# Justin900429/autonomous_driving_with_diffusion_model

Measured on AMD Instinct MI355X. Metric: denoising-steps/sec, higher is better.
Workload: dtype f32

## Files before the change

### autonomous_driving_with_diffusion_model_amd/_lib.py

```python
from __future__ import annotations

import ctypes as C
import os
from typing import Optional, Sequence

import torch

_HERE = os.path.dirname(os.path.abspath(__file__))
LIB_PATH = os.environ.get("ADX_LIB") or os.path.join(_HERE, "libadx.so")

c_f32p = C.POINTER(C.c_float)
i32, i64, f32, vp = C.c_int32, C.c_int64, C.c_float, C.c_void_p


class TConvDesc(C.Structure):
    _fields_ = [("kind", i32), ("taps", i32), ("stride", i32), ("pad", i32), ("c0", i32), ("c1", i32),
                ("cout", i32), ("lin", i32), ("lout", i32), ("groups", i32), ("eps", f32), ("w_layout", i32),
                ("w_flip", i32), ("exact", i32), ("lin_valid", i32), ("lout_valid", i32)]


class TConvIO(C.Structure):
    _fields_ = [("x0", vp), ("x0_sb", i64), ("x0_sc", i64), ("x0_sl", i64),
                ("x1", vp), ("x1_sb", i64), ("x1_sc", i64), ("x1_sl", i64),
                ("packed_w", vp), ("bias", vp), ("gamma", vp), ("beta", vp),
# ... 151 lines not shown
    "adx_dpm_step": (i32, [C.POINTER(DpmCoef), vp, vp, vp, vp, vp, i32, i32, i32, vp]),
    "adx_traj_select": (i32, [C.POINTER(SelectCfg), vp, vp, vp, vp, vp, vp]),
    "adx_control_state_bytes": (C.c_size_t, [i32, i32, i32]),
    "adx_control_step": (i32, [C.POINTER(ControlCfg), vp, vp, vp, vp, vp, vp]),
    "adx_control_reset": (i32, [vp, i32, i32, i32, vp, vp]),
    "adx_noise_normal": (i32, [vp, i32, i64, vp, i64, vp]),
    "adx_noise_words": (i32, [vp, i32, i64, vp, i64, vp]),
    "adx_noise_advance": (i32, [vp, vp]),
    "adx_warm_init": (i32, [vp, i32, vp, vp, i32, i32, i32, i32, f32, f32, vp, i64, i32, vp]),
    "adx_add_noise": (i32, [vp, vp, vp, vp, vp, i32, vp, i32, i32, i32, i32, vp]),
}

_LAZY_SIGS = {
    "adx_conv2d_pack_ds": (i32, [i32, i32, vp, vp, vp]),
    "adx_conv2d_block_s2_cells": (i32, [i32, i32, vp, vp, vp, vp, vp, vp, vp, vp, vp, i32, i32, i32, i32, vp]),
}

EXPORTED_SYMBOLS = tuple(_SIGS) + tuple(_LAZY_SIGS)

_lib: Optional[C.CDLL] = None


class AdxError(RuntimeError):
    pass


class AdxRangeError(AdxError):

    def __init__(self, groups):
        self.groups = list(groups)
# ... 92 lines not shown
```

### autonomous_driving_with_diffusion_model_amd/csrc/adx_common.h

```cpp
#pragma once
#include <atomic>
#include <mutex>
#include <hip/hip_runtime.h>
#include <stdint.h>
#include <stdio.h>
#include <string.h>

#include "../../include/adx.h"
#include "plan.h"

namespace adx {

void set_error(const char* fmt, ...);

#define ADX_CHECK_HIP(expr)                                                              \
  do {                                                                                   \
    hipError_t _e = (expr);                                                              \
    if (_e != hipSuccess) {                                                              \
      adx::set_error("%s failed: %s (%s:%d)", #expr, hipGetErrorString(_e), __FILE__, __LINE__); \
      return ADX_ERR_HIP;                                                                \
    }                                                                                    \
  } while (0)

#define ADX_REQUIRE(cond, ...)                                                           \
// ... 16 lines not shown
struct DebugSwitches {
  bool conv_exact = false;
  bool wgrad_exact = false;
  bool tconv_exact = false;
  bool unet_chain = true;
  unsigned chain_mask = ~0u;
  bool unet_pipe = true;
  bool conv_vrow = true;
  bool conv_cells = true;
  int train_cells = 5;
  int hs_mode = -1;
  bool wgrad_deterministic = false;
  bool hs_dma = true;
  bool hs_s2q = true;
  bool hs_persist = true;
  int resnet_streams = 2;
  int resnet_split_from = -1;
  bool check_range = false;
};
const DebugSwitches& debug_switches();

struct DeviceOnce {
  std::atomic<uint64_t>& done;
  uint64_t bit = 0;
  bool owner = false;
  static std::mutex& mu() { static std::mutex m; return m; }
  explicit DeviceOnce(std::atomic<uint64_t>& d) : done(d) {
    int dev = 0;
    (void)hipGetDevice(&dev);
    bit = 1ull << (dev & 63);
// ... 46 lines not shown
```

### autonomous_driving_with_diffusion_model_amd/csrc/api.cpp

```cpp
#include <stdarg.h>
#include <stdlib.h>

#include "tconv.h"

namespace adx {

static thread_local char g_err[512] = "";

void set_error(const char* fmt, ...) {
  va_list ap;
  va_start(ap, fmt);
  vsnprintf(g_err, sizeof(g_err), fmt, ap);
  va_end(ap);
}

static thread_local PlanSink* t_plan_sink = nullptr;
PlanSink* plan_sink() { return t_plan_sink; }
void plan_set_sink(PlanSink* s) { t_plan_sink = s; }

int plan_emit(PlanSink* s, const PlanLaunch& l) {
  ADX_REQUIRE(s->n < s->cap, "plan export: more than %d launches", s->cap);
  s->rec[s->n++] = l;
  return ADX_OK;
}
// ... 11 lines not shown
  static const DebugSwitches sw = [] {
    DebugSwitches d;
    auto is = [](const char* name, char v) { const char* e = getenv(name); return e != nullptr && e[0] == v && e[1] == '\0'; };
    d.conv_exact = is("ADX_CONV_EXACT", '1');
    d.wgrad_exact = is("ADX_WGRAD_EXACT", '1');
    d.tconv_exact = is("ADX_TCONV_EXACT", '1');
    d.unet_chain = !is("ADX_UNET_CHAIN", '0');
    d.unet_pipe = !is("ADX_UNET_PIPE", '0');
    d.conv_cells = !is("ADX_CONV_CELLS", '0');
    d.conv_vrow = !is("ADX_CONV_VROW", '0');
    d.train_cells = is("ADX_TRAIN_CELLS", '0') ? 0 : (is("ADX_TRAIN_CELLS", '1') ? 1 : (is("ADX_TRAIN_CELLS", '2') ? 2 : (is("ADX_TRAIN_CELLS", '3') ? 3 : (is("ADX_TRAIN_CELLS", '4') ? 4 : 5))));
    d.check_range = is("ADX_CHECK_RANGE", '1');
    d.hs_dma = !is("ADX_HS_DMA", '0');
    d.hs_persist = !is("ADX_HS_PERSIST", '0');
    d.hs_s2q = !is("ADX_HS_S2Q", '0');
    d.wgrad_deterministic = is("ADX_WGRAD_DETERMINISTIC", '1');
    if (const char* e = getenv("ADX_CHAIN_MASK")) d.chain_mask = (unsigned)strtoul(e, nullptr, 0);
    if (const char* e = getenv("ADX_HS_MODE")) d.hs_mode = atoi(e);
    if (const char* e = getenv("ADX_RESNET_SPLIT_FROM")) d.resnet_split_from = atoi(e) < 0 ? -1 : atoi(e);
    if (const char* e = getenv("ADX_RESNET_STREAMS")) d.resnet_streams = atoi(e) < 1 ? 1 : (atoi(e) > 4 ? 4 : atoi(e));
    return d;
  }();
  return sw;
}

int embed_forward(const adx_embed_weights* w, int dim, const int64_t* t, int t_rows, const float* cond,
                  const float* feat, int feat_rows, int rows, float* time_embed, float* mish_cond, hipStream_t s);
int ddim_step(const adx_step_coef* c, const float* mo, const float* x, const float* z, const float* tgt,
              const float* mask, float* prev, float* x0, int b, int h, int d, hipStream_t s);
int ddpm_step(const adx_step_coef* c, const float* mo, const float* x, const float* z, const float* tgt,
// ... 151 lines not shown
```

### autonomous_driving_with_diffusion_model_amd/csrc/conv2d.hip

```cpp
#include <stdlib.h>

#include <vector>

#include "adx_common.h"
#include "conv2d_internal.h"

namespace adx {

constexpr int kCoutT = 64;
constexpr size_t kMaxLds = 96 * 1024;

template <int STRIDE, int K, int ROWS, int CCH = 16>
__global__ void __launch_bounds__(256) conv2d_kernel(const Conv2dArgs a) {
  constexpr int TH = 4 * ROWS;
  constexpr int CC = (K == 7) ? 4 : CCH;
  constexpr int PH = (TH - 1) * STRIDE + K;
  constexpr int PW = (kTileW - 1) * STRIDE + K;
  constexpr int PLANE = PH * PW;
  constexpr int NP = CC * PLANE;
  constexpr int PITEMS = (NP + 255) / 256;
  constexpr int NTAPS = K * K;
  constexpr int NW4 = NTAPS * CC * (kCoutT / 4);
  constexpr int WITEMS = (NW4 + 255) / 256;
  extern __shared__ __attribute__((aligned(16))) float smem[];
// ... 375 lines not shown
    ADX_REQUIRE(scale == nullptr && relu == 0, "conv2d: BatchNorm-backward statistics belong to data-gradient launches");
    a.bs_raw = bst->raw; a.bs_out = bst->out; a.bs_mean = bst->mean; a.bs_rstd = bst->rstd; a.bs_gamma = bst->gamma;
    a.bs_beta = bst->beta; a.bs_mask = bst->mask; a.bs_bits = bst->mask == 1 ? bst->bits : nullptr;
    a.res_bits = bst->res_bits;
  }
  a.x_cells = (fmt & kFmtXCells) != 0; a.y_cells = (fmt & kFmtYCells) != 0; a.res_cells = (fmt & kFmtResCells) != 0 && res != nullptr;
  Hs3x3Query q;
  q.N = N; q.H = H; q.W = W; q.fmt = fmt;
  q.stats_floats = stats_part != nullptr && stats_p != nullptr ? stats_floats : 0;
  q.bst_mask = a.bs_mask; q.bst_bits = a.bs_bits != nullptr;
  q.x_scale = x_amax == nullptr ? kXScaleNone : (x_amax_n < 0 ? kXScalePre : kXScaleDynamic);
  q.affine = scale != nullptr; q.relu = relu != 0; q.has_res = res != nullptr;
  q.y_aligned = (reinterpret_cast<uintptr_t>(y) & 15) == 0; q.res_aligned = (reinterpret_cast<uintptr_t>(res) & 15) == 0;
  q.split_floats = t_split_floats;
  if (L.k == 3 && L.stride == 1) {
    const int rc = device_cus(&q.cus);
    if (rc != ADX_OK) return rc;
  }
  const Hs3x3Plan plan = conv2d_hs3x3_plan(L, q);
  ADX_REQUIRE(a.res_bits == nullptr || (res != nullptr && L.dgrad && plan.stats == 2),
              "conv2d: a masked residual belongs to a data-gradient launch with the statistics epilogue");
  ADX_REQUIRE(plan.admitted, "conv2d: the cell layout belongs to plain launches of the pipelined 3x3 kernel (%d -> %d, k%d s%d)", L.cin, L.cout,
              L.k, L.stride);
  if (conv2d_hs_eligible(L)) {
    if (plan.stats != 0) {
      a.stats_part = stats_part;
      a.stats_p = plan.stats_tiles;
      *stats_p = plan.stats_tiles;
    }
    return conv2d_hs_launch(L, a, s, &plan);
  }
// ... 83 lines not shown
}

int adx_conv2d_forward_cells(const adx_conv2d_desc* d, const void* x, const float* packed_w, const float* scale,
                             const float* shift, const void* res, void* y, int32_t n, int32_t h, int32_t w, int32_t relu,
                             int32_t fmt, adx_stream stream) {
  ConvSpec L;
  int rc = spec_from_desc(d, &L);
  if (rc != ADX_OK) return rc;
  ADX_REQUIRE(x && packed_w && y, "adx_conv2d_forward_cells: null tensor");
  ADX_REQUIRE((scale == nullptr) == (shift == nullptr), "adx_conv2d_forward_cells: scale and shift go together");
  ADX_REQUIRE(fmt >= 0 && fmt <= 7 && (fmt & kFmtYCells), "adx_conv2d_forward_cells: fmt %d (the output is a cell tensor)", fmt);
  ADX_REQUIRE(conv2d_hs3x3_plain(L, n, h, w), "adx_conv2d_forward_cells: not a plain launch of the pipelined 3x3 kernel "
              "(adx_conv2d_cells_supported)");
  return conv2d_launch_raw(L, (const float*)x, packed_w, scale, shift, (const float*)res, (float*)y, n, h, w, relu,
                           (hipStream_t)stream, nullptr, 0, nullptr, 0, nullptr, fmt);
}

static int block_s2_specs(int32_t cin, int32_t cout, ConvSpec* c1, ConvSpec* ds, const char* who) {
  const adx_conv2d_desc d1{cin, cout, 3, 2, 1}, dd{cin, cout, 1, 2, 0};
  int rc = spec_from_desc(&d1, c1);
  if (rc == ADX_OK) rc = spec_from_desc(&dd, ds);
  if (rc != ADX_OK) return rc;
  ADX_REQUIRE(resnet_fuses_ds(*c1, *ds), "%s: %d -> %d is no block entry the split-fp16 kernels fuse (cin %% 16, cout %% 64, not ADX_CONV_EXACT=1)",
              who, cin, cout);
  return ADX_OK;
}

int adx_conv2d_pack_ds(int32_t cin, int32_t cout, const float* w, float* packed, adx_stream stream) {
  ConvSpec c1, ds;
  const int rc = block_s2_specs(cin, cout, &c1, &ds, "adx_conv2d_pack_ds");
// ... 472 lines not shown
```

### autonomous_driving_with_diffusion_model_amd/csrc/conv2d_hs.hip

```cpp
#include <type_traits>
#include <stdlib.h>

#include "adx_common.h"
#include "conv2d_internal.h"
#include "conv2d_hs_common.h"

namespace adx {

template <bool AFFINE = true>
__device__ __forceinline__ void cells_store32(float (&v)[16], const float* sc, const float* sh, int cl0, const float (*res8)[8],
                                              bool relu, __amdgpu_buffer_rsrc_t yrsrc, uint32_t vcell, uint32_t so, uint32_t cplane,
                                              float& amax) {
  float lm = 0.f;
#pragma unroll
  for (int i = 0; i < 2; ++i)
#pragma unroll
    for (int j = 0; j < 4; ++j) {
      const auto sw = __builtin_amdgcn_permlane32_swap(f2u(v[8 * i + j]), f2u(v[8 * i + 4 + j]), false, false);
      v[8 * i + j] = u2f(sw[0]);
      v[8 * i + 4 + j] = u2f(sw[1]);
    }
#pragma unroll
  for (int i = 0; i < 2; ++i) {
    float o[8];
// ... 1539 lines not shown
  const bool in_ok = (size_t)N * L.cin * q.H * q.W * sizeof(float) < 0xC0000000u;
  const bool bytes_ok = in_ok && (size_t)N * L.cout * OH * OW * sizeof(float) < 0xC0000000u;
  const bool vfits = (long)N * (OW + 1) < (1L << 21);
  const int vw = N > 1 ? OW + 1 : OW;
  const int vtiles_x = (int)(((long)N * vw - (N > 1 ? 1 : 0) + kTileW - 1) / kTileW);
  const bool vrow_ok = sw.conv_vrow && N > 1 && vfits && bytes_ok;
  const bool q_shape = sw.hs_mode < 0 && L.cout % 128 == 0 && L.cin_pad % 64 == 0;
  const bool q_fp32out = q_shape && xc && !yc && !rc && !q.affine && vfits && bytes_ok;
  const bool q_train = q_fp32out && sw.train_cells >= 3 && !q.has_res && q.x_scale == kXScaleNone && q.bst_mask == 0;
  const bool q_dgrad = q_fp32out && sw.train_cells >= 5 && xscaled && !q.relu && (q.bst_mask == 2 || (q.bst_mask == 1 && q.bst_bits));
  const bool q_plain = q_shape && xc && yc && (!q.has_res || rc) && q.x_scale == kXScaleNone;
  const int stats_tiles = q_train || q_dgrad ? ceil_div(OH, kQTH) * vtiles_x
                                             : ceil_div(OH, th) * (!yc && !rc && vrow_ok ? vtiles_x : N * ceil_div(OW, kTileW));
  p.stats_need = (size_t)stats_tiles * (L.cout * 2 + L.cout / 64);
  const bool stats = q.stats_floats > 0 && p.stats_need <= q.stats_floats;
  const bool split_shape = mode == 0 && grid0 <= 64 && nchunks >= 8;
  if (q.fmt == kFmtXCells && q.stats_floats > 0 && q.bst_mask == 0 && q.x_scale == kXScaleNone && sw.train_cells != 0 && !L.dgrad)
    p.admitted = in_ok && stats;
  else if (q.fmt == (kFmtXCells | kFmtXScaled) && L.dgrad && xscaled && sw.train_cells >= 4)
    p.admitted = in_ok;
  else if (q.fmt != 0)
    p.admitted = q.stats_floats == 0 && sw.conv_cells && !L.dgrad && bytes_ok && !split_shape;

  p.family = kHs3x3; p.mode = mode; p.threads = mode == 0 ? 256 : 512;
  p.tiles_x = ceil_div(OW, kTileW); p.tiles_y = ceil_div(OH, th); p.cout_tiles = L.cout / (kHsCout * ct);
  p.vw = OW; p.cper = nchunks;
  p.grid = (size_t)p.cout_tiles * p.tiles_x * p.tiles_y * N;
  if (stats) { p.stats = q.bst_mask != 0 ? 2 : 1; p.stats_tiles = stats_tiles; }
  if (!stats && split_shape && q.split_floats > 0 && q.x_scale == kXScaleNone && (OH * OW) % 4 == 0 && q.y_aligned && (!q.has_res || q.res_aligned)) {
    const size_t out_floats = (size_t)N * L.cout * OH * OW;
    int S = 16;
    while (S > 1 && (nchunks % S != 0 || (nchunks / S) % 2 != 0 || p.grid * S > 256 || out_floats * S > q.split_floats)) S >>= 1;
    if (S > 1) { p.ksplit = S; p.cper = nchunks / S; p.grid *= S; }
  }
  const bool cells_out = !stats && p.ksplit == 1 && (xc || yc || rc) && !(xc && xscaled && !yc && !rc);
  if (stats ? q_train || q_dgrad : cells_out && q_plain) {
    p.family = kHs3x3q; p.dma = sw.hs_dma; p.threads = kQNT;
    p.lds = p.dma ? kQLdsD : kQLds;
    p.vw = vw; p.tiles_x = vtiles_x; p.tiles_y = ceil_div(OH, kQTH); p.cout_tiles = L.cout / 128;
    p.q_slots = ceil_div(p.tiles_x * p.tiles_y, 8);
    if (sw.hs_dma && sw.hs_persist) p.q_slots = std::min(p.q_slots, std::max(1, q.cus / (8 * p.cout_tiles)));
    p.grid = (size_t)8 * p.cout_tiles * p.q_slots;
    return p;
  }
  p.lds = hs3x3_lds(mode, p.stats);
  if (p.ksplit > 1) return p;
  p.xcells = xc; p.ycells = cells_out;
  p.vr = !cells_out && (!(xc || yc || rc) || ((stats || xscaled) && !yc && !rc)) && vrow_ok;
  if (p.ycells || p.vr) {
    p.vw = vw; p.tiles_x = vtiles_x;
// ... 101 lines not shown
  a.KH = 2; a.KW = 2; a.stride = 1; a.pad = 0; a.relu = 0;
  a.cin_pad = cout; a.cc = kHsCC;
  a.d2s_cin = cin; a.d2s_h = H; a.d2s_w = W;
  ADX_REQUIRE((size_t)cin * H * W * sizeof(float) < 0x7FFFFFFFu, "conv2d_hs_dgrad_s2: one image of dx exceeds the 32-bit byte offsets");
  return hs_launch_t<1, 2, 2, 2, false>(a, s);
}

int conv2d_hs_launch(const ConvSpec& L, Conv2dArgs a, hipStream_t s, const Hs3x3Plan* plan) {
  ADX_REQUIRE((size_t)L.cin * a.H * a.W * sizeof(float) < 0xC0000000u, "conv2d_hs: one image of the input exceeds the 32-bit byte offsets");
  const bool ds = a.w_ds != nullptr;
  if (hs_is_stem(L) && !ds) {
    ADX_REQUIRE(a.x_amax == nullptr && a.res == nullptr, "conv2d_hs stem: no residual / dynamic range");
    return hs_stem_launch(a, s);
  }
  if (L.k == 3 && L.stride == 1 && !ds) {
    if (plan != nullptr && plan->family != kHsNone) return plan->family == kHs3x3q ? conv2d_hs3x3q_launch(*plan, a, s) : hs3x3_launch(*plan, a, s);
    ADX_REQUIRE(a.stats_part == nullptr, "conv2d_hs: statistics requested from a launch the pipelined kernel does not serve");
    return hs_launch_t<1, 3, 2, 2, false>(a, s);
  }
  if (L.k == 3 && L.stride == 2 && L.pad == 1) {
    if (a.x_cells || a.y_cells) {
      ADX_REQUIRE(ds && a.x_amax == nullptr && a.res == nullptr && a.d2s_cin == 0,
                  "conv2d_hs: cell-layout operands of the stride-2 conv need the fused downsample launch (no residual, no dynamic range)");
      if (a.x_cells && a.y_cells) return hs_launch_t<2, 3, 1, 1, true, true, true>(a, s);
      return a.x_cells ? hs_launch_t<2, 3, 1, 1, true, true, false>(a, s) : hs_launch_t<2, 3, 1, 1, true, false, true>(a, s);
    }
    return ds ? hs_launch_t<2, 3, 1, 1, true>(a, s) : hs_launch_t<2, 3, 1, 1, false>(a, s);
  }
  set_error("conv2d_hs: no kernel for k=%d stride=%d pad=%d%s", L.k, L.stride, L.pad, ds ? " with a fused downsample" : "");
  return ADX_ERR_INVALID;
// ... 10 lines not shown
```

### autonomous_driving_with_diffusion_model_amd/csrc/conv2d_hs16.hip

```cpp
#include "adx_common.h"
#include "conv2d_internal.h"
#include "conv2d_hs_common.h"

namespace adx {

namespace {

typedef __attribute__((address_space(3))) void lds_void;

__device__ __forceinline__ f32x4 mfma16(f16x8 a, f16x8 b, f32x4 c) { return __builtin_amdgcn_mfma_f32_16x16x32_f16(a, b, c, 0, 0, 0); }

__device__ __forceinline__ void half4(uint32_t h0, uint32_t h1, uint32_t l0, uint32_t l1, float* out) {
  const float inv = 1.f / kLoScale;
  asm("v_fma_mix_f32 %0, %1, %2, %3 op_sel:[0,0,0] op_sel_hi:[1,0,1]" : "=v"(out[0]) : "v"(l0), "s"(inv), "v"(h0));
  asm("v_fma_mix_f32 %0, %1, %2, %3 op_sel:[1,0,1] op_sel_hi:[1,0,1]" : "=v"(out[1]) : "v"(l0), "s"(inv), "v"(h0));
  asm("v_fma_mix_f32 %0, %1, %2, %3 op_sel:[0,0,0] op_sel_hi:[1,0,1]" : "=v"(out[2]) : "v"(l1), "s"(inv), "v"(h1));
  asm("v_fma_mix_f32 %0, %1, %2, %3 op_sel:[1,0,1] op_sel_hi:[1,0,1]" : "=v"(out[3]) : "v"(l1), "s"(inv), "v"(h1));
}

}

template <bool DMA, int TRAIN = 0>
__global__ void __launch_bounds__(kQNT, 2) conv2d_hs3x3q_kernel(const Conv2dArgs a) {
  constexpr bool S2 = TRAIN == 3;
// ... 565 lines not shown
      const uint32_t so = cell0 + (uint32_t)(2 * cb) * 2u * cplane;
      __builtin_amdgcn_raw_buffer_store_b128(hi, yrsrc, vcell[rr], so, 0);
      __builtin_amdgcn_raw_buffer_store_b128(lo, yrsrc, vcell[rr], so + cplane, 0);
      asm volatile("s_nop 0" ::"v"(hi), "v"(lo));
    }
  bad |= ((vcell[0] != kOutside) & out_of_fp16(am[0])) | ((vcell[1] != kOutside) & out_of_fp16(am[1]));
  } while (S2 && ++pass < 2);
  }
  if (!has_next) break;
  if constexpr (TRAIN == 1 || TRAIN == 2) __syncthreads();
  sp = sp_next; tx = ntx; ty = nty; oy0 = n_oy0; vx0 = n_vx0;
  }
  range_flag(a.status, bad);
}

int conv2d_hs3x3q_launch(const Hs3x3Plan& p, Conv2dArgs a, hipStream_t s) {
  typedef void (*QKernel)(const Conv2dArgs);
  static const QKernel table[2][3] = {
      {&conv2d_hs3x3q_kernel<false, 0>, &conv2d_hs3x3q_kernel<false, 1>, &conv2d_hs3x3q_kernel<false, 2>},
      {&conv2d_hs3x3q_kernel<true, 0>, &conv2d_hs3x3q_kernel<true, 1>, &conv2d_hs3x3q_kernel<true, 2>}};
  static std::atomic<uint64_t> attr{0};
  if (DeviceOnce once{attr}; once) {
    for (int dma = 0; dma < 2; ++dma)
      for (const QKernel k : table[dma])
        ADX_CHECK_HIP(hipFuncSetAttribute(reinterpret_cast<const void*>(k), hipFuncAttributeMaxDynamicSharedMemorySize, (int)(dma ? kQLdsD : kQLds)));
    once.commit();
  }
  ADX_REQUIRE((long)a.N * p.vw < (1L << 21), "conv2d_hs: batch x width exceeds the virtual-row arithmetic");
  const size_t tiles = (size_t)p.cout_tiles * p.tiles_x * p.tiles_y;
  ADX_REQUIRE(tiles < (1u << 31), "conv2d_hs: grid too large");
// ... 13 lines not shown
  if (DeviceOnce once{attr}; once) {
    ADX_CHECK_HIP(hipFuncSetAttribute(reinterpret_cast<const void*>(&conv2d_hs3x3q_kernel<true, 3>), hipFuncAttributeMaxDynamicSharedMemorySize, (int)kQLdsS2));
    once.commit();
  }
  ADX_REQUIRE(p.q && a.x_cells && a.y_cells && a.w_ds != nullptr && a.y_ds != nullptr && a.res == nullptr && a.x_amax == nullptr,
              "conv2d_hs: the 16x16x32 block entry takes a cell input, two cell outputs, no residual and no dynamic range");
  a.vw = p.vw; a.inv_vw = 1.f / (float)p.vw;
  a.tiles_x = p.tiles_x; a.tiles_y = p.tiles_y; a.cout_tiles = p.cout_tiles; a.ntiles = p.cout_tiles * p.tiles_x * p.tiles_y;
  a.q_slots = p.q_slots;
  a.ksplit = 1; a.cper = a.cin_pad / kHsCC; a.part = nullptr;
  conv2d_hs3x3q_kernel<true, 3><<<dim3((unsigned)p.grid), dim3(p.threads), p.lds, s>>>(a);
  ADX_LAUNCH_CHECK();
  return ADX_OK;
}

}
```

### autonomous_driving_with_diffusion_model_amd/csrc/conv2d_hs_common.h

```cpp
#pragma once
#include "adx_common.h"

namespace adx {

typedef _Float16 f16x8 __attribute__((ext_vector_type(8)));
typedef uint32_t u32x4 __attribute__((ext_vector_type(4)));
typedef _Float16 f16x2 __attribute__((ext_vector_type(2)));

constexpr int kHsCout = 64;
constexpr int kHsCC = 16;
constexpr float kLoScale = 2048.f;

constexpr int kQNT = 512;
constexpr int kQTH = 8;
constexpr int kQPW = 34;
constexpr int kQPlane = (kQTH + 2) * kQPW;
constexpr int kQPlaneP = 344;
constexpr int kQPairs = 4 * kQPlane;
constexpr int kQPit = (kQPairs + kQNT - 1) / kQNT;
constexpr int kQWst = 1024;
constexpr size_t kQLds = (size_t)2 * 8 * kQPlaneP * 16 + (size_t)2 * kQWst * 16 + 256 * sizeof(float) + 2 * 16 + 512 * sizeof(float);
constexpr int kQPlaneD = 352;
constexpr int kQPairsD = 4 * kQPlaneD;
constexpr size_t kQLdsD = (size_t)2 * 8 * kQPlaneD * 16 + (size_t)2 * kQWst * 16 + 256 * sizeof(float) + 2 * 16 + 512 * sizeof(float) +
                          (size_t)kQPit * kQNT * sizeof(uint32_t);
constexpr size_t kQLdsS2 = kQLdsD + (size_t)4 * kQPit * kQNT * sizeof(uint32_t);
static_assert(kQLds <= 160 * 1024 && kQLdsD <= 160 * 1024 && kQLdsS2 <= 160 * 1024, "LDS budget");

#ifdef ADX_HS_M16_TIMING
typedef float f32x4_t __attribute__((ext_vector_type(4)));
__device__ __forceinline__ f32x16 hs_mfma(f16x8 a, f16x8 b, f32x16 c) {
  f32x4_t c0 = __builtin_shufflevector(c, c, 0, 1, 2, 3), c1 = __builtin_shufflevector(c, c, 4, 5, 6, 7);
  c0 = __builtin_amdgcn_mfma_f32_16x16x32_f16(a, b, c0, 0, 0, 0);
  c1 = __builtin_amdgcn_mfma_f32_16x16x32_f16(a, b, c1, 0, 0, 0);
  c[0] = c0[0]; c[1] = c0[1]; c[2] = c0[2]; c[3] = c0[3];
  c[4] = c1[0]; c[5] = c1[1]; c[6] = c1[2]; c[7] = c1[3];
  return c;
}
#else
__device__ __forceinline__ f32x16 hs_mfma(f16x8 a, f16x8 b, f32x16 c) { return __builtin_amdgcn_mfma_f32_32x32x16_f16(a, b, c, 0, 0, 0); }
#endif

// ... 20 lines not shown
```

### autonomous_driving_with_diffusion_model_amd/csrc/conv2d_internal.h

```cpp
#pragma once
#include <vector>

#include "adx_common.h"

namespace adx {

constexpr int kTileH = 4;
constexpr int kTileW = 32;

struct ConvSpec {
  int cin, cout, k, stride, pad;
  int t_w, t_g, t_b, t_m, t_v;
  size_t o_w, o_scale, o_shift;
  int cin_pad, cc;
  int fuse_with;
  int dgrad;
};

struct Conv2dArgs {
  const float* x;
  const float* w;
  const float* scale;
  const float* shift;
  const float* res;
// ... 45 lines not shown
  hipStream_t side[kMaxSub - 1] = {nullptr, nullptr, nullptr};
  hipEvent_t ev_fork = nullptr, ev_join[kMaxSub - 1] = {nullptr, nullptr, nullptr};
  int side_device = -1;
  uint32_t* status = nullptr;
};

namespace adx {

struct BnBwdStats { const float* raw; const float* out; const float* mean; const float* rstd; const float* gamma; const float* beta; int mask;
                    const uint8_t* bits = nullptr; const uint8_t* res_bits = nullptr; };
int conv2d_launch_raw(const ConvSpec& L, const float* x, const float* w, const float* scale, const float* shift,
                      const float* res, float* y, int N, int H, int W, int relu, hipStream_t s,
                      const uint32_t* x_amax = nullptr, int x_amax_n = 0, float* stats_part = nullptr, size_t stats_floats = 0,
                      int* stats_p = nullptr, int fmt = 0, const BnBwdStats* bst = nullptr);

enum { kHsNone = 0, kHs3x3 = 1, kHs3x3q = 2 };
enum { kXScaleNone = 0, kXScaleDynamic = 1, kXScalePre = 2 };
struct Hs3x3Query {
  int N = 0, H = 0, W = 0;
  int fmt = 0;
  size_t stats_floats = 0;
  int bst_mask = 0;
  bool bst_bits = false;
  int x_scale = kXScaleNone;
  bool affine = false, relu = false, has_res = false;
  bool y_aligned = true, res_aligned = true;
  size_t split_floats = 0;
  int cus = 0;
};
struct Hs3x3Plan {
  bool admitted = false;
  int family = kHsNone;
  int mode = 0;
  int stats = 0;
  bool xcells = false, ycells = false, vr = false;
  bool dma = false;
  int ksplit = 1, cper = 0;
  int tiles_x = 0, tiles_y = 0, cout_tiles = 0, vw = 0, q_slots = 0;
  size_t grid = 0;
  int threads = 0;
  size_t lds = 0;
  int stats_tiles = 0;
  size_t stats_need = 0;
// ... 20 lines not shown
  q.fmt = x_cells ? kFmtXCells | kFmtXScaled : 0;
  q.x_scale = x_cells ? kXScalePre : kXScaleDynamic;
  const Hs3x3Plan p = conv2d_hs3x3_plan(L, q);
  return L.dgrad && p.admitted && p.stats == 2;
}
int conv2d_pack_raw(const float* w, float* packed, int cout, int cin, int k, int cin_pad, int dgrad, hipStream_t s);
int conv2d_pack_spec(const ConvSpec& consumer, const float* w, float* packed, int dgrad, hipStream_t s);
bool conv2d_hs_eligible(const ConvSpec& L, const DebugSwitches& sw = debug_switches());
size_t conv2d_packed_floats(const ConvSpec& L);
int conv2d_hs_pack(const ConvSpec& consumer, const float* w, void* packed, int dgrad, hipStream_t s);
struct HsPackJob { const float* w; void* packed; int cout, cin_pad, cin, taps, dgrad; };
bool conv2d_hs_pack_batchable(const ConvSpec& consumer, int dgrad);
int conv2d_hs_pack_many(const HsPackJob* jobs, int n, hipStream_t s);
int conv2d_hs_launch(const ConvSpec& L, Conv2dArgs a, hipStream_t s, const Hs3x3Plan* plan = nullptr);
int conv2d_hs3x3q_launch(const Hs3x3Plan& p, Conv2dArgs a, hipStream_t s);
bool conv2d_hs_dgrad_s2_eligible(int cin, int cout);
int conv2d_hs_dgrad_s2(const float* w, const float* dy, float* dx, int accumulate, int N, int cin, int cout, int H, int W,
                       float* wbuild, float* wimg, const uint32_t* dy_amax, int dy_amax_n, hipStream_t s);
void conv2d_set_split_scratch(float* p, size_t floats);
void conv2d_set_status(uint32_t* word);
uint32_t* conv2d_status();
int conv2d_hs_stem_pool(const ConvSpec& L, const float* x, const float* w, const float* scale, const float* shift,
                        float* pooled, int N, int H, int W, hipStream_t s, const uint8_t* frames_u8 = nullptr,
                        const float* mean = nullptr, const float* stdv = nullptr, int y_cells = 0);
int conv2d_hs_launch_block_s2(const ConvSpec& c1, const ConvSpec& ds, const float* x, const float* w1, const float* scale1,
                              const float* shift1, float* y1, const float* wd, const float* scaled, const float* shiftd,
                              float* yd, int N, int H, int W, hipStream_t s, int x_cells = 0, int y_cells = 0, int relu = 1,
                              bool force_32 = false);
struct HsS2Query {
  int N = 0, H = 0, W = 0;
// ... 74 lines not shown
```

### include/adx.h

```cpp
#ifndef ADX_H
#define ADX_H

#include <stddef.h>
#include <stdint.h>

#ifdef __cplusplus
extern "C" {
#endif

#define ADX_OK 0
#define ADX_ERR_INVALID (-1)
#define ADX_ERR_HIP (-2)
#define ADX_ERR_STATE (-3)
#define ADX_ERR_RANGE (-4)

typedef void* adx_stream;

int adx_version(void);
const char* adx_source_hash(void);
const char* adx_last_error(void);


typedef struct adx_tconv_desc {
  int32_t kind, taps, stride, pad;
// ... 134 lines not shown
                             int32_t max_records);
int32_t adx_resnet_status_words(const adx_resnet* r);
int adx_resnet_set_status(adx_resnet* r, uint32_t* words );
const char* adx_resnet_status_name(const adx_resnet* r, int32_t group);

typedef struct adx_conv2d_desc { int32_t cin, cout, k, stride, pad; } adx_conv2d_desc;
size_t adx_conv2d_packed_bytes(const adx_conv2d_desc* d);
int adx_conv2d_pack(const adx_conv2d_desc* d, const float* w , float* packed, adx_stream s);
int adx_conv2d_forward(const adx_conv2d_desc* d, const float* x, const float* packed_w, const float* scale,
                       const float* shift, const float* res, float* y, int32_t n, int32_t h, int32_t w,
                       int32_t relu, adx_stream s);
int adx_conv2d_cells_supported(const adx_conv2d_desc* d, int32_t n, int32_t h, int32_t w);
int adx_conv2d_forward_cells(const adx_conv2d_desc* d, const void* x, const float* packed_w, const float* scale,
                             const float* shift, const void* res, void* y, int32_t n, int32_t h, int32_t w, int32_t relu,
                             int32_t fmt, adx_stream s);
int adx_conv2d_pack_ds(int32_t cin, int32_t cout, const float* w, float* packed, adx_stream s);
int adx_conv2d_block_s2_cells(int32_t cin, int32_t cout, const void* x, const float* packed_w1, const float* scale1,
                              const float* shift1, void* y1, const float* packed_wd, const float* scaled, const float* shiftd,
                              void* yd, int32_t n, int32_t h, int32_t w, int32_t flags, adx_stream s);
int adx_conv2d_stem_pool(const void* x, int32_t x_u8, const float* packed_w, const float* scale, const float* shift,
                         const float* mean, const float* stdv, void* y, int32_t n, int32_t h, int32_t w, int32_t y_cells,
                         adx_stream s);
size_t adx_conv2d_wgrad_scratch_bytes(void);
int adx_conv2d_wgrad(const adx_conv2d_desc* d, const float* x, const float* dy, float* dw, int32_t n, int32_t h,
                     int32_t w, void* scratch, adx_stream s);
int adx_conv2d_wgrad_ex(const adx_conv2d_desc* d, const float* x, const float* dy, float* dw, int32_t n, int32_t h,
                        int32_t w, void* scratch, int32_t estimate_range, adx_stream s);
int adx_conv2d_wgrad_cells(const adx_conv2d_desc* d, const void* x_cells, const void* dy_cells, const float* dy_scale, float* dw,
                           int32_t n, int32_t h, int32_t w, void* scratch, adx_stream s);

// ... 167 lines not shown
```

Before: 167.2.

## Add 4-wave two-workgroups-per-CU 3x3 cell conv kernel variant

Adds a new 256-thread form of the fp16-split 3x3 stride-1 cell-layout convolution. It uses a smaller LDS footprint so two workgroups fit per CU, and each workgroup computes 64 output channels with a persistent tile loop that prefetches the next tile's patch. The planner picks it for plain all-cell inference launches with enough tiles, based on a queried occupancy. A plan-query API is also exposed. The aim is better latency hiding and CU utilisation on the ResNet perception convs, at the cost of another kernel path with different tiling.

```diff
diff --git a/autonomous_driving_with_diffusion_model_amd/_lib.py b/autonomous_driving_with_diffusion_model_amd/_lib.py
--- a/autonomous_driving_with_diffusion_model_amd/_lib.py
+++ b/autonomous_driving_with_diffusion_model_amd/_lib.py
@@ -189,6 +189,7 @@
 _LAZY_SIGS = {
     "adx_conv2d_pack_ds": (i32, [i32, i32, vp, vp, vp]),
     "adx_conv2d_block_s2_cells": (i32, [i32, i32, vp, vp, vp, vp, vp, vp, vp, vp, vp, i32, i32, i32, i32, vp]),
+    "adx_conv2d_cells_plan": (i32, [i32, i32, i32, i32, i32, i32, i32, i32, C.POINTER(i32)]),
 }
 
 EXPORTED_SYMBOLS = tuple(_SIGS) + tuple(_LAZY_SIGS)
diff --git a/autonomous_driving_with_diffusion_model_amd/csrc/adx_common.h b/autonomous_driving_with_diffusion_model_amd/csrc/adx_common.h
--- a/autonomous_driving_with_diffusion_model_amd/csrc/adx_common.h
+++ b/autonomous_driving_with_diffusion_model_amd/csrc/adx_common.h
@@ -54,6 +54,7 @@
   bool hs_dma = true;
   bool hs_s2q = true;
   bool hs_persist = true;
+  int hs_q64 = 1;
   int resnet_streams = 2;
   int resnet_split_from = -1;
   bool check_range = false;
diff --git a/autonomous_driving_with_diffusion_model_amd/csrc/api.cpp b/autonomous_driving_with_diffusion_model_amd/csrc/api.cpp
--- a/autonomous_driving_with_diffusion_model_amd/csrc/api.cpp
+++ b/autonomous_driving_with_diffusion_model_amd/csrc/api.cpp
@@ -49,6 +49,7 @@
     d.hs_dma = !is("ADX_HS_DMA", '0');
     d.hs_persist = !is("ADX_HS_PERSIST", '0');
     d.hs_s2q = !is("ADX_HS_S2Q", '0');
+    d.hs_q64 = is("ADX_HS_Q64", '0') ? 0 : (is("ADX_HS_Q64", '2') ? 2 : 1);
     d.wgrad_deterministic = is("ADX_WGRAD_DETERMINISTIC", '1');
     if (const char* e = getenv("ADX_CHAIN_MASK")) d.chain_mask = (unsigned)strtoul(e, nullptr, 0);
     if (const char* e = getenv("ADX_HS_MODE")) d.hs_mode = atoi(e);
diff --git a/autonomous_driving_with_diffusion_model_amd/csrc/conv2d.hip b/autonomous_driving_with_diffusion_model_amd/csrc/conv2d.hip
--- a/autonomous_driving_with_diffusion_model_amd/csrc/conv2d.hip
+++ b/autonomous_driving_with_diffusion_model_amd/csrc/conv2d.hip
@@ -413,7 +413,8 @@
   q.y_aligned = (reinterpret_cast<uintptr_t>(y) & 15) == 0; q.res_aligned = (reinterpret_cast<uintptr_t>(res) & 15) == 0;
   q.split_floats = t_split_floats;
   if (L.k == 3 && L.stride == 1) {
-    const int rc = device_cus(&q.cus);
+    int rc = device_cus(&q.cus);
+    if (rc == ADX_OK && debug_switches().hs_q64 != 0) rc = conv2d_hs3x3q64_wgs_per_cu(&q.q64_wgs_per_cu);
     if (rc != ADX_OK) return rc;
   }
   const Hs3x3Plan plan = conv2d_hs3x3_plan(L, q);
@@ -527,6 +528,25 @@
               "(adx_conv2d_cells_supported)");
   return conv2d_launch_raw(L, (const float*)x, packed_w, scale, shift, (const float*)res, (float*)y, n, h, w, relu,
                            (hipStream_t)stream, nullptr, 0, nullptr, 0, nullptr, fmt);
+}
+
+int adx_conv2d_cells_plan(int32_t cin, int32_t cout, int32_t n, int32_t h, int32_t w, int32_t has_res, int32_t cus,
+                          int32_t wgs_per_cu, int32_t* ints) {
+  ADX_REQUIRE(ints != nullptr && n >= 1 && h >= 1 && w >= 1 && cus >= 1 && wgs_per_cu >= 0, "adx_conv2d_cells_plan: bad argument");
+  const adx_conv2d_desc d{cin, cout, 3, 1, 1};
+  ConvSpec L;
+  const int rc = spec_from_desc(&d, &L);
+  if (rc != ADX_OK) return rc;
+  Hs3x3Query q;
+  q.N = n; q.H = h; q.W = w; q.has_res = has_res != 0;
+  q.fmt = kFmtXCells | kFmtYCells | (has_res ? kFmtResCells : 0);
+  q.cus = cus > 8 ? cus : 8; q.q64_wgs_per_cu = wgs_per_cu;
+  const Hs3x3Plan p = conv2d_hs3x3_plan(L, q);
+  const bool cell_launch = p.admitted && p.family != kHsNone;
+  const int32_t v[ADX_CONV3X3_PLAN_INTS] = {cell_launch ? p.family : kHsNone, p.mode, p.threads, (int32_t)p.grid, p.q_slots, (int32_t)p.lds,
+                                            p.tiles_x, p.tiles_y, p.cout_tiles};
+  for (int i = 0; i < ADX_CONV3X3_PLAN_INTS; ++i) ints[i] = cell_launch ? v[i] : 0;
+  return ADX_OK;
 }
 
 static int block_s2_specs(int32_t cin, int32_t cout, ConvSpec* c1, ConvSpec* ds, const char* who) {
diff --git a/autonomous_driving_with_diffusion_model_amd/csrc/conv2d_hs.hip b/autonomous_driving_with_diffusion_model_amd/csrc/conv2d_hs.hip
--- a/autonomous_driving_with_diffusion_model_amd/csrc/conv2d_hs.hip
+++ b/autonomous_driving_with_diffusion_model_amd/csrc/conv2d_hs.hip
@@ -1577,7 +1577,10 @@
                                              : ceil_div(OH, th) * (!yc && !rc && vrow_ok ? vtiles_x : N * ceil_div(OW, kTileW));
   p.stats_need = (size_t)stats_tiles * (L.cout * 2 + L.cout / 64);
   const bool stats = q.stats_floats > 0 && p.stats_need <= q.stats_floats;
-  const bool split_shape = mode == 0 && grid0 <= 64 && nchunks >= 8;
+  const bool q64_scope = sw.hs_q64 != 0 && sw.hs_mode < 0 && sw.hs_dma && sw.conv_cells && L.cout % 64 == 0 && L.cin_pad % 64 == 0 && !L.dgrad &&
+                         q.stats_floats == 0 && xc && yc && (!q.has_res || rc) && q.x_scale == kXScaleNone && bytes_ok && vfits;
+  const bool q64_forced = sw.hs_q64 == 2 && q64_scope;
+  const bool split_shape = mode == 0 && grid0 <= 64 && nchunks >= 8 && !q64_forced;
   if (q.fmt == kFmtXCells && q.stats_floats > 0 && q.bst_mask == 0 && q.x_scale == kXScaleNone && sw.train_cells != 0 && !L.dgrad)
     p.admitted = in_ok && stats;
   else if (q.fmt == (kFmtXCells | kFmtXScaled) && L.dgrad && xscaled && sw.train_cells >= 4)
@@ -1597,6 +1600,16 @@
     if (S > 1) { p.ksplit = S; p.cper = nchunks / S; p.grid *= S; }
   }
   const bool cells_out = !stats && p.ksplit == 1 && (xc || yc || rc) && !(xc && xscaled && !yc && !rc);
+  const long q64_tiles = (long)vtiles_x * ceil_div(OH, kQTH) * (L.cout / 64);
+  if (q64_scope && p.ksplit == 1 && q.q64_wgs_per_cu >= 2 && (q64_forced || (!q_plain && q64_tiles >= 2L * q.cus))) {
+    p.family = kHs3x3q64; p.dma = true; p.threads = kQ64NT;
+    p.lds = kQ64Lds;
+    p.vw = vw; p.tiles_x = vtiles_x; p.tiles_y = ceil_div(OH, kQTH); p.cout_tiles = L.cout / 64;
+    p.q_slots = ceil_div(p.tiles_x * p.tiles_y, 8);
+    if (sw.hs_persist) p.q_slots = std::min(p.q_slots, std::max(1, q.q64_wgs_per_cu * q.cus / (8 * p.cout_tiles)));
+    p.grid = (size_t)8 * p.cout_tiles * p.q_slots;
+    return p;
+  }
   if (stats ? q_train || q_dgrad : cells_out && q_plain) {
     p.family = kHs3x3q; p.dma = sw.hs_dma; p.threads = kQNT;
     p.lds = p.dma ? kQLdsD : kQLds;
@@ -1728,6 +1741,7 @@
     return hs_stem_launch(a, s);
   }
   if (L.k == 3 && L.stride == 1 && !ds) {
+    if (plan != nullptr && plan->family == kHs3x3q64) return conv2d_hs3x3q64_launch(*plan, a, s);
     if (plan != nullptr && plan->family != kHsNone) return plan->family == kHs3x3q ? conv2d_hs3x3q_launch(*plan, a, s) : hs3x3_launch(*plan, a, s);
     ADX_REQUIRE(a.stats_part == nullptr, "conv2d_hs: statistics requested from a launch the pipelined kernel does not serve");
     return hs_launch_t<1, 3, 2, 2, false>(a, s);
diff --git a/autonomous_driving_with_diffusion_model_amd/csrc/conv2d_hs16.hip b/autonomous_driving_with_diffusion_model_amd/csrc/conv2d_hs16.hip
--- a/autonomous_driving_with_diffusion_model_amd/csrc/conv2d_hs16.hip
+++ b/autonomous_driving_with_diffusion_model_amd/csrc/conv2d_hs16.hip
@@ -603,6 +603,236 @@
   range_flag(a.status, bad);
 }
 
+namespace q64 {
+
+template <bool DMA, int TRAIN = 0>
+__global__ void __launch_bounds__(kQ64NT, 2) conv2d_hs3x3q_kernel(const Conv2dArgs a) {
+  static_assert(DMA && TRAIN == 0, "the 4-wave form serves the LDS-DMA inference launch only");
+  constexpr int NT = kQ64NT, PW = kQPW, PLANE = kQPlaneD, PP = kQPlaneD, PIT = kQ64Pit, WST = kQ64Wst, NPAIRS = kQPairsD;
+  constexpr int GST = PP, PLST = 4 * PP;
+  extern __shared__ __attribute__((aligned(16))) unsigned char smem_raw[];
+  u32x4* patch = reinterpret_cast<u32x4*>(smem_raw);
+  u32x4* wl = patch + 8 * PP;
+  float* ss = reinterpret_cast<float*>(wl + 2 * WST);
+  u32x4* dummy = reinterpret_cast<u32x4*>(ss + 128);
+  uint32_t* gnext = reinterpret_cast<uint32_t*>(dummy + 2);
+  const int tid = threadIdx.x, lane = tid & 63;
+  const int rowpair = __builtin_amdgcn_readfirstlane(tid >> 6);
+  const int j = lane & 15, kq = lane >> 4;
+  const int Qs = a.q_slots;
+  const int xcd = blockIdx.x & 7, rr_ = blockIdx.x >> 3;
+  const int ct = rr_ % a.cout_tiles, slot = rr_ / a.cout_tiles;
+  const int nsp = a.tiles_x * a.tiles_y;
+  const int sp_end = (int)(((long)(xcd + 1) * nsp) >> 3);
+  int sp = (int)(((long)xcd * nsp) >> 3) + slot;
+  if (sp >= sp_end) return;
+  int ty = sp / a.tiles_x, tx = sp - ty * a.tiles_x;
+  int oy0 = ty * kQTH, vx0 = tx * 32;
+  auto vdiv = [&](int v) { return (int)(((float)v + 0.5f) * a.inv_vw); };
+  const size_t hw = (size_t)a.H * a.W;
+  const int nch16 = a.cin_pad / 16, nch32 = a.cin_pad / 32, nstages = nch32 * 9;
+  constexpr uint32_t kOutside = 0xC0000000u;
+  const __amdgpu_buffer_rsrc_t xrsrc = __builtin_amdgcn_make_buffer_rsrc(
+      const_cast<float*>(a.x), 0, (int)(uint32_t)((size_t)a.N * a.Cin * hw * sizeof(float)), 0x00020000);
+  const uint32_t plane_bytes = (uint32_t)(hw * sizeof(float));
+  auto goff_of = [&](int t_, int k, int oy0_, int vx0_) -> uint32_t {
+    const int e = t_ + NT * k;
+    const int g = e / PLANE, p = e - g * PLANE;
+    const int py = p / PW, px = p - py * PW;
+    const int iy = oy0_ - 1 + py;
+    const int v = vx0_ - 1 + px;
+    const int ni = vdiv(v < 0 ? 0 : v);
+    const int ix = v - ni * a.vw;
+    const bool ok = e < NPAIRS && p < kQPlane && iy >= 0 && iy < a.H && ix >= 0 && ix < a.W && ni < a.N;
+    return !ok ? kOutside : (uint32_t)((size_t)ni * a.Cin * hw * sizeof(float) + (size_t)g * 8 * hw * sizeof(float) + ((size_t)iy * a.W + ix) * 16);
+  };
+  uint32_t goff[PIT];
+#pragma unroll
+  for (int k = 0; k < PIT; ++k) goff[k] = goff_of(tid, k, oy0, vx0);
+  const u32x4* wsrc = reinterpret_cast<const u32x4*>(a.w);
+  int wsrc_off[2];
+#pragma unroll
+  for (int k = 0; k < 2; ++k) wsrc_off[k] = ((ct * nch16 + k) * 9) * 256 + tid;
+  float ssv = 0.f;
+  if (tid < 128) {
+    const int c = ct * 64 + (tid & 63);
+    ssv = a.scale == nullptr ? (tid < 64 ? 1.f : 0.f) : (tid < 64 ? a.scale[c] : a.shift[c]);
+  }
+
+  f32x4 accm[4][4], accl[4][4];
+
+  const int wcell = __builtin_amdgcn_readfirstlane(tid & ~63);
+  auto load_w = [&](int stage, int buf) {
+    const int chunk = stage / 9, tap = stage - chunk * 9;
+    const u32x4* ws = wsrc + (size_t)(chunk * 18 + tap) * 256;
+#pragma unroll
+    for (int k = 0; k < 2; ++k) __builtin_amdgcn_global_load_lds(ws + wsrc_off[k], (lds_void*)(wl + buf * WST + wcell + NT * k), 16, 0, 0);
+  };
+  auto load_p_at = [&](int chunk, int k, uint32_t go) {
+    const uint32_t cbase = (uint32_t)chunk * 32u * plane_bytes;
+    if (k < PIT - 1 || wcell + NT * k < NPAIRS) {
+      u32x4* d = patch + wcell + NT * k;
+      __builtin_amdgcn_raw_ptr_buffer_load_lds(xrsrc, (lds_void*)d, 16, go, cbase, 0, 0);
+      __builtin_amdgcn_raw_ptr_buffer_load_lds(xrsrc, (lds_void*)(d + PLST), 16, go, cbase + 4 * plane_bytes, 0, 0);
+    }
+  };
+
+  load_w(0, 0);
+#pragma unroll
+  for (int k = 0; k < PIT; ++k) load_p_at(0, k, goff[k]);
+  if (tid < 128) ss[tid] = ssv;
+  asm volatile("s_waitcnt vmcnt(0)" ::: "memory");
+  __syncthreads();
+
+  bool bad = false;
+  for (;;) {
+  int zero_ = 0;
+  asm volatile("" : "+s"(zero_));
+  const int tl = tid + zero_;
+#pragma unroll
+  for (int k = 0; k < PIT; ++k) goff[k] = goff_of(tl, k, oy0, vx0);
+#pragma unroll
+  for (int k = 0; k < 2; ++k) wsrc_off[k] = ((ct * nch16 + k) * 9) * 256 + tl;
+  const int j_l = tl & 15, kq_l = (tl & 63) >> 4;
+  const int pb_lane = kq_l * GST + (rowpair * 2) * PW + j_l;
+  const int wa_lane = (kq_l >> 1) * 256 + (kq_l & 1) * 64 + j_l;
+  const int sp_next = sp + Qs;
+  const bool has_next = sp_next < sp_end;
+  const int nty = sp_next / a.tiles_x, ntx = sp_next - nty * a.tiles_x;
+  const int n_oy0 = nty * kQTH, n_vx0 = ntx * 32;
+  if (has_next) {
+#pragma unroll
+    for (int k = 0; k < PIT; ++k) gnext[k * NT + tid] = goff_of(tl, k, n_oy0, n_vx0);
+  }
+#pragma unroll
+  for (int cb = 0; cb < 4; ++cb)
+#pragma unroll
+    for (int pb = 0; pb < 4; ++pb)
+#pragma unroll
+      for (int i = 0; i < 4; ++i) { accm[cb][pb][i] = 0.f; accl[cb][pb][i] = 0.f; }
+
+  for (int cp = 0; cp < nch32; cp += 2) {
+#pragma unroll
+    for (int i = 0; i < 18; ++i) {
+      const int s = 9 * cp + i;
+      const int cpar = i / 9, t = i % 9, kh = t / 3, kw = t % 3;
+      const u32x4* pb0 = patch + pb_lane + kh * PW + kw;
+      const u32x4* wa0 = wl + (i & 1) * WST + wa_lane;
+      load_w(s + 1 < nstages ? s + 1 : (has_next ? 0 : nstages - 1), (i + 1) & 1);
+      __builtin_amdgcn_sched_barrier(0);
+      f16x8 A[2][4], B[2][4];
+#pragma unroll
+      for (int pl = 0; pl < 2; ++pl) {
+#pragma unroll
+        for (int cb = 0; cb < 4; ++cb) A[pl][cb] = __builtin_bit_cast(f16x8, wa0[pl * 128 + cb * 16]);
+#pragma unroll
+        for (int pb = 0; pb < 4; ++pb) B[pl][pb] = __builtin_bit_cast(f16x8, pb0[pl * PLST + (pb >> 1) * PW + (pb & 1) * 16]);
+      }
+#pragma unroll
+      for (int pb = 0; pb < 4; ++pb) {
+#pragma unroll
+        for (int cb = 0; cb < 4; ++cb) {
+          accm[cb][pb] = mfma16(A[0][cb], B[0][pb], accm[cb][pb]);
+          accl[cb][pb] = mfma16(A[0][cb], B[1][pb], accl[cb][pb]);
+        }
+#pragma unroll
+        for (int cb = 0; cb < 4; ++cb) accl[cb][pb] = mfma16(A[1][cb], B[0][pb], accl[cb][pb]);
+      }
+      asm volatile("s_waitcnt vmcnt(0)" ::: "memory");
+      __syncthreads();
+      if (t == 8) {
+        const bool tile_end = cpar == 1 && cp + 2 >= nch32;
+        if (!tile_end) {
+#pragma unroll
+          for (int k = 0; k < PIT; ++k) load_p_at(cp + cpar + 1, k, goff[k]);
+          asm volatile("s_waitcnt vmcnt(0)" ::: "memory");
+          __syncthreads();
+        } else if (has_next) {
+#pragma unroll
+          for (int k = 0; k < PIT; ++k) load_p_at(0, k, gnext[k * NT + tid]);
+        }
+      }
+    }
+  }
+
+  {
+  const int rw = kq;
+  const int vcol = vx0 + 16 * (rw & 1) + j;
+  const int nl = vdiv(vcol), xl = vcol - nl * a.vw;
+  const bool col_valid = nl < a.N && xl < a.W;
+  const uint32_t plane_ob = (uint32_t)(a.OH * a.OW) * (uint32_t)sizeof(float);
+  const uint32_t cplane = (uint32_t)(a.OH * a.OW) * 16u;
+  const uint32_t img_bytes = (uint32_t)a.N * (uint32_t)a.Cout * plane_ob;
+  const uint32_t img_off = (uint32_t)nl * (uint32_t)a.Cout * plane_ob;
+  const __amdgpu_buffer_rsrc_t yrsrc = __builtin_amdgcn_make_buffer_rsrc(a.y, 0, (int)img_bytes, 0x00020000);
+  const __amdgpu_buffer_rsrc_t rrsrc = __builtin_amdgcn_make_buffer_rsrc(
+      const_cast<float*>(a.res != nullptr ? a.res : a.y), 0, a.res != nullptr ? (int)img_bytes : 0, 0x00020000);
+  const int cout0 = ct * 64;
+  const uint32_t cell0 = (uint32_t)(cout0 >> 3) * 2u * cplane;
+  uint32_t vcell[2];
+#pragma unroll
+  for (int rr = 0; rr < 2; ++rr) {
+    const int oy = oy0 + rowpair * 2 + rr;
+    vcell[rr] = (col_valid && oy < a.OH) ? img_off + (uint32_t)(oy * a.OW + xl) * 16u + (uint32_t)(rw >> 1) * 2u * cplane : kOutside;
+  }
+  u32x4 rh[4][2], rl[4][2];
+#pragma unroll
+  for (int cb = 0; cb < 4; ++cb)
+#pragma unroll
+    for (int rr = 0; rr < 2; ++rr) {
+      const uint32_t so = cell0 + (uint32_t)(2 * cb) * 2u * cplane;
+      rh[cb][rr] = __builtin_amdgcn_raw_buffer_load_b128(rrsrc, vcell[rr], so, 0);
+      rl[cb][rr] = __builtin_amdgcn_raw_buffer_load_b128(rrsrc, vcell[rr], so + cplane, 0);
+    }
+  const float* sc = ss;
+  const float* sh = ss + 64;
+  float am[2] = {0.f, 0.f};
+#pragma unroll
+  for (int cb = 0; cb < 4; ++cb)
+#pragma unroll
+    for (int rr = 0; rr < 2; ++rr) {
+      float x[4], y[4];
+#pragma unroll
+      for (int i = 0; i < 4; ++i) {
+        const int cl = cb * 16 + 4 * kq + i;
+        x[i] = (accm[cb][2 * rr][i] + accl[cb][2 * rr][i] * (1.f / kLoScale)) * sc[cl] + sh[cl];
+        y[i] = (accm[cb][2 * rr + 1][i] + accl[cb][2 * rr + 1][i] * (1.f / kLoScale)) * sc[cl] + sh[cl];
+      }
+      float o[8];
+#pragma unroll
+      for (int i = 0; i < 4; ++i) {
+        const auto sw = __builtin_amdgcn_permlane16_swap(f2u(x[i]), f2u(y[i]), false, false);
+        o[i] = u2f(sw[0]);
+        o[4 + i] = u2f(sw[1]);
+      }
+      float r8[8];
+      half4(rh[cb][rr][0], rh[cb][rr][1], rl[cb][rr][0], rl[cb][rr][1], r8);
+      half4(rh[cb][rr][2], rh[cb][rr][3], rl[cb][rr][2], rl[cb][rr][3], r8 + 4);
+#pragma unroll
+      for (int i = 0; i < 8; ++i) {
+        const float tsum = o[i] + r8[i];
+        o[i] = a.relu ? __builtin_fmaxf(tsum, 0.f) : tsum;
+        am[rr] = fp16_amax(am[rr], o[i]);
+      }
+      u32x4 hi, lo;
+      split8(o, 1.f, hi, lo);
+      const uint32_t so = cell0 + (uint32_t)(2 * cb) * 2u * cplane;
+      __builtin_amdgcn_raw_buffer_store_b128(hi, yrsrc, vcell[rr], so, 0);
+      __builtin_amdgcn_raw_buffer_store_b128(lo, yrsrc, vcell[rr], so + cplane, 0);
+      asm volatile("s_nop 0" ::"v"(hi), "v"(lo));
+    }
+  bad |= ((vcell[0] != kOutside) & out_of_fp16(am[0])) | ((vcell[1] != kOutside) & out_of_fp16(am[1]));
+  }
+  if (!has_next) break;
+  asm volatile("s_waitcnt vmcnt(0)" ::: "memory");
+  __syncthreads();
+  sp = sp_next; tx = ntx; ty = nty; oy0 = n_oy0; vx0 = n_vx0;
+  }
+  range_flag(a.status, bad);
+}
+
+}
+
 int conv2d_hs3x3q_launch(const Hs3x3Plan& p, Conv2dArgs a, hipStream_t s) {
   typedef void (*QKernel)(const Conv2dArgs);
   static const QKernel table[2][3] = {
@@ -646,4 +876,43 @@
   return ADX_OK;
 }
 
+static std::atomic<uint64_t> g_q64_once{0};
+static std::atomic<int> g_q64_wgs[64];
+int conv2d_hs3x3q64_wgs_per_cu(int* wgs) {
+  int dev = 0;
+  ADX_CHECK_HIP(hipGetDevice(&dev));
+  if (DeviceOnce once{g_q64_once}; once) {
+    const void* k = reinterpret_cast<const void*>(&q64::conv2d_hs3x3q_kernel<true, 0>);
+    ADX_CHECK_HIP(hipFuncSetAttribute(k, hipFuncAttributeMaxDynamicSharedMemorySize, (int)kQ64Lds));
+    int n = 0;
+    ADX_CHECK_HIP(hipOccupancyMaxActiveBlocksPerMultiprocessor(&n, k, kQ64NT, kQ64Lds));
+    g_q64_wgs[dev & 63].store(n, std::memory_order_relaxed);
+    once.commit();
+  }
+  *wgs = g_q64_wgs[dev & 63].load(std::memory_order_relaxed);
+  return ADX_OK;
 }
+
+int conv2d_hs3x3q64_launch(const Hs3x3Plan& p, Conv2dArgs a, hipStream_t s) {
+  int wgs = 0;
+  const int rc = conv2d_hs3x3q64_wgs_per_cu(&wgs);
+  if (rc != ADX_OK) return rc;
+  ADX_REQUIRE(p.family == kHs3x3q64 && p.dma && p.stats == 0 && a.x_cells && a.y_cells && (a.res == nullptr || a.res_cells) && a.x_amax == nullptr &&
+                  a.Cout % 64 == 0 && a.cin_pad % 64 == 0 && a.Cin == a.cin_pad,
+              "conv2d_hs: the 4-wave 16x16x32 form takes plain all-cell launches with Cout %% 64 == 0 and Cin %% 64 == 0");
+  ADX_REQUIRE((long)a.N * p.vw < (1L << 21), "conv2d_hs: batch x width exceeds the virtual-row arithmetic");
+  const size_t tiles = (size_t)p.cout_tiles * p.tiles_x * p.tiles_y;
+  ADX_REQUIRE(tiles < (1u << 31) && p.cout_tiles == a.Cout / 64 && p.q_slots >= 1 && p.grid == (size_t)8 * p.cout_tiles * p.q_slots,
+              "conv2d_hs: inconsistent plan of the 4-wave 16x16x32 form");
+  ADX_REQUIRE((size_t)a.N * a.Cout * a.OH * a.OW * sizeof(float) < 0xC0000000u && (size_t)a.N * a.Cin * a.H * a.W * sizeof(float) < 0xC0000000u,
+              "conv2d_hs: a cell-layout tensor exceeds the 32-bit byte offsets");
+  a.vw = p.vw; a.inv_vw = 1.f / (float)p.vw;
+  a.tiles_x = p.tiles_x; a.tiles_y = p.tiles_y; a.cout_tiles = p.cout_tiles; a.ntiles = (int)tiles;
+  a.q_slots = p.q_slots;
+  a.ksplit = 1; a.cper = a.cin_pad / kHsCC; a.part = nullptr;
+  q64::conv2d_hs3x3q_kernel<true, 0><<<dim3((unsigned)p.grid), dim3(p.threads), p.lds, s>>>(a);
+  ADX_LAUNCH_CHECK();
+  return ADX_OK;
+}
+
+}
diff --git a/autonomous_driving_with_diffusion_model_amd/csrc/conv2d_hs_common.h b/autonomous_driving_with_diffusion_model_amd/csrc/conv2d_hs_common.h
--- a/autonomous_driving_with_diffusion_model_amd/csrc/conv2d_hs_common.h
+++ b/autonomous_driving_with_diffusion_model_amd/csrc/conv2d_hs_common.h
@@ -26,6 +26,13 @@
                           (size_t)kQPit * kQNT * sizeof(uint32_t);
 constexpr size_t kQLdsS2 = kQLdsD + (size_t)4 * kQPit * kQNT * sizeof(uint32_t);
 static_assert(kQLds <= 160 * 1024 && kQLdsD <= 160 * 1024 && kQLdsS2 <= 160 * 1024, "LDS budget");
+
+constexpr int kQ64NT = 256;
+constexpr int kQ64Pit = (kQPairsD + kQ64NT - 1) / kQ64NT;
+constexpr int kQ64Wst = 512;
+constexpr size_t kQ64Lds = (size_t)8 * kQPlaneD * 16 + (size_t)2 * kQ64Wst * 16 + 128 * sizeof(float) + 2 * 16 +
+                           (size_t)kQ64Pit * kQ64NT * sizeof(uint32_t);
+static_assert(kQ64Lds == 68128 && 2 * kQ64Lds <= 160 * 1024, "two workgroups of the 4-wave form share a CU's 160 KB of LDS");
 
 #ifdef ADX_HS_M16_TIMING
 typedef float f32x4_t __attribute__((ext_vector_type(4)));
diff --git a/autonomous_driving_with_diffusion_model_amd/csrc/conv2d_internal.h b/autonomous_driving_with_diffusion_model_amd/csrc/conv2d_internal.h
--- a/autonomous_driving_with_diffusion_model_amd/csrc/conv2d_internal.h
+++ b/autonomous_driving_with_diffusion_model_amd/csrc/conv2d_internal.h
@@ -83,7 +83,7 @@
                       const uint32_t* x_amax = nullptr, int x_amax_n = 0, float* stats_part = nullptr, size_t stats_floats = 0,
                       int* stats_p = nullptr, int fmt = 0, const BnBwdStats* bst = nullptr);
 
-enum { kHsNone = 0, kHs3x3 = 1, kHs3x3q = 2 };
+enum { kHsNone = 0, kHs3x3 = 1, kHs3x3q = 2, kHs3x3q64 = 3 };
 enum { kXScaleNone = 0, kXScaleDynamic = 1, kXScalePre = 2 };
 struct Hs3x3Query {
   int N = 0, H = 0, W = 0;
@@ -96,6 +96,7 @@
   bool y_aligned = true, res_aligned = true;
   size_t split_floats = 0;
   int cus = 0;
+  int q64_wgs_per_cu = 0;
 };
 struct Hs3x3Plan {
   bool admitted = false;
@@ -146,6 +147,8 @@
 int conv2d_hs_pack_many(const HsPackJob* jobs, int n, hipStream_t s);
 int conv2d_hs_launch(const ConvSpec& L, Conv2dArgs a, hipStream_t s, const Hs3x3Plan* plan = nullptr);
 int conv2d_hs3x3q_launch(const Hs3x3Plan& p, Conv2dArgs a, hipStream_t s);
+int conv2d_hs3x3q64_launch(const Hs3x3Plan& p, Conv2dArgs a, hipStream_t s);
+int conv2d_hs3x3q64_wgs_per_cu(int* wgs);
 bool conv2d_hs_dgrad_s2_eligible(int cin, int cout);
 int conv2d_hs_dgrad_s2(const float* w, const float* dy, float* dx, int accumulate, int N, int cin, int cout, int H, int W,
                        float* wbuild, float* wimg, const uint32_t* dy_amax, int dy_amax_n, hipStream_t s);
diff --git a/include/adx.h b/include/adx.h
--- a/include/adx.h
+++ b/include/adx.h
@@ -172,6 +172,9 @@
 int adx_conv2d_forward_cells(const adx_conv2d_desc* d, const void* x, const float* packed_w, const float* scale,
                              const float* shift, const void* res, void* y, int32_t n, int32_t h, int32_t w, int32_t relu,
                              int32_t fmt, adx_stream s);
+#define ADX_CONV3X3_PLAN_INTS 9
+int adx_conv2d_cells_plan(int32_t cin, int32_t cout, int32_t n, int32_t h, int32_t w, int32_t has_res, int32_t cus,
+                          int32_t wgs_per_cu, int32_t* ints);
 int adx_conv2d_pack_ds(int32_t cin, int32_t cout, const float* w, float* packed, adx_stream s);
 int adx_conv2d_block_s2_cells(int32_t cin, int32_t cout, const void* x, const float* packed_w1, const float* scale1,
                               const float* shift1, void* y1, const float* packed_wd, const float* scaled, const float* shiftd,
```

New measurement: 167.1. No clear change (-0.0%).
